# ForJadeForest/DistillCLIP

Hardware: AMD Instinct MI355X
Metric: image-text pairs/sec (distill step) (higher is better)
Workload: dtype bf16

## Files before the change

distillclip_amd/csrc/common.h:

```cpp
#pragma once
#include <hip/hip_runtime.h>
#include <stdint.h>

typedef __bf16 bf16_t;
typedef __attribute__((ext_vector_type(8))) __bf16 bf16x8;
typedef __attribute__((ext_vector_type(4))) __bf16 bf16x4;
typedef __attribute__((ext_vector_type(2))) __bf16 bf16x2;
typedef __attribute__((ext_vector_type(8))) _Float16 f16x8;
typedef __attribute__((ext_vector_type(4))) _Float16 f16x4;
typedef __attribute__((ext_vector_type(4))) short s16x4;
typedef __attribute__((ext_vector_type(4))) float f32x4;
typedef __attribute__((ext_vector_type(16))) float f32x16;
typedef __attribute__((ext_vector_type(4))) unsigned int u32x4;

#include "dclip.h"

void dclip_set_error(const char* fmt, ...);

#define DCLIP_REQUIRE(cond, ...)                 \
    do {                                          \
        if (!(cond)) {                            \
            dclip_set_error(__VA_ARGS__);         \
            return DCLIP_EINVAL;                  \
        }                                         \
// ... 20 lines not shown
    hipError_t e = hipGetLastError();
    if (e != hipSuccess) {
        dclip_explain_hip_error(what, (int)e, hipGetErrorString(e));
        return DCLIP_ELAUNCH;
    }
    return DCLIP_OK;
}

__device__ __forceinline__ float bf2f(bf16_t x) { return (float)x; }
__device__ __forceinline__ bf16_t f2bf(float x) { return (bf16_t)x; }

__device__ __forceinline__ float wave_sum(float v) {
#pragma unroll
    for (int o = 32; o > 0; o >>= 1) v += __shfl_xor(v, o);
    return v;
}
__device__ __forceinline__ float wave_max(float v) {
#pragma unroll
    for (int o = 32; o > 0; o >>= 1) v = fmaxf(v, __shfl_xor(v, o));
    return v;
}

__device__ __forceinline__ float quick_gelu_f(float x) { return x * __builtin_amdgcn_rcpf(1.f + __expf(-1.702f * x)); }
__device__ __forceinline__ float erf_tail(float ax_over_sqrt2, float phi) {
    const float t = __builtin_amdgcn_rcpf(fmaf(0.3275911f, ax_over_sqrt2, 1.f));
    float p = fmaf(1.061405429f, t, -1.453152027f);
    p = fmaf(p, t, 1.421413741f);
    p = fmaf(p, t, -0.284496736f);
    p = fmaf(p, t, 0.254829592f);
    return p * t * phi;
}
__device__ __forceinline__ float gelu_erf_f(float x) {
    const float phi = __expf(-0.5f * x * x);
    const float tail = erf_tail(fabsf(x) * 0.70710678118654752f, phi);
    const float cdf = x >= 0.f ? 1.f - 0.5f * tail : 0.5f * tail;
    return x * cdf;
}
__device__ __forceinline__ float dgelu_erf_f(float x) {
    const float phi = __expf(-0.5f * x * x);
    const float tail = erf_tail(fabsf(x) * 0.70710678118654752f, phi);
    const float cdf = x >= 0.f ? 1.f - 0.5f * tail : 0.5f * tail;
    return fmaf(x * phi, 0.3989422804014327f, cdf);
}

__device__ __forceinline__ void gelu_erf_both_f(float x, float& g, float& dg) {
    const float phi = __expf(-0.5f * x * x);
    const float tail = erf_tail(fabsf(x) * 0.70710678118654752f, phi);
    const float cdf = x >= 0.f ? 1.f - 0.5f * tail : 0.5f * tail;
    g = x * cdf;
    dg = fmaf(x * phi, 0.3989422804014327f, cdf);
}

#define DCLIP_DG_LO (-0.13f)
#define DCLIP_DG_STEP (1.26f / 255.f)
__device__ __forceinline__ unsigned dg_pack4(float a, float b, float c, float d) {
    const float inv = 255.f / 1.26f, off = 0.13f * (255.f / 1.26f);
    unsigned r = 0;
    r = __builtin_amdgcn_cvt_pk_u8_f32(__builtin_rintf(fmaf(a, inv, off)), 0, r);
    r = __builtin_amdgcn_cvt_pk_u8_f32(__builtin_rintf(fmaf(b, inv, off)), 1, r);
    r = __builtin_amdgcn_cvt_pk_u8_f32(__builtin_rintf(fmaf(c, inv, off)), 2, r);
    r = __builtin_amdgcn_cvt_pk_u8_f32(__builtin_rintf(fmaf(d, inv, off)), 3, r);
    return r;
}
__device__ __forceinline__ float dg_unpack(unsigned w, int byte) {
    return fmaf((float)((w >> (8 * byte)) & 0xffu), DCLIP_DG_STEP, DCLIP_DG_LO);
}

__device__ __forceinline__ int xcd_remap(int bid, int nwg) {
    const int q = nwg >> 3, r = nwg & 7, x = bid & 7;
// ... 3 lines not shown
```

distillclip_amd/csrc/encoder.cpp:

```cpp
#include <math.h>
#include <stdlib.h>
#include <string.h>
#include <atomic>
#include <new>
#include <vector>
#include "common.h"

namespace {

#define CK(expr)                      \
    do {                              \
        int _rc = (expr);             \
        if (_rc != DCLIP_OK) return _rc; \
    } while (0)

inline size_t up256(size_t x) { return (x + 255) & ~(size_t)255; }

struct Bump {
    char* base; size_t off;
    explicit Bump(void* b) : base((char*)b), off(0) {}
    template <class T> T* take(size_t n) {
        T* p = base ? (T*)(base + off) : nullptr;
        off += up256(n * sizeof(T));
        return p;
// ... 300 lines not shown
        dclip_set_error("dclip_encoder: clearing the backward seeds failed");
        return DCLIP_ELAUNCH;
    }
    return DCLIP_OK;
}

static int encoder_forward_impl(const dclip_encoder* e, const void* input, const bf16_t* ext_patches, int64_t B, const void* const* params,
                                const void* wcache, void* workspace, size_t ws_bytes, int training,
                                float* last_representation, float* const* rep_out, float* emb_out, int64_t tokens_eff,
                                void* st) {
    DCLIP_REQUIRE(e && (input || ext_patches) && params && wcache && workspace && last_representation, "dclip_encoder_forward: null argument");
    DCLIP_REQUIRE(B > 0, "dclip_encoder_forward: empty batch");
    const Plan& p = e->p;
    DCLIP_REQUIRE(!ext_patches || (p.image && ((uintptr_t)ext_patches % 16) == 0), "dclip_encoder_forward_patches: image towers only, 16-byte aligned rows");
    DCLIP_REQUIRE(!training || p.train, "dclip_encoder_forward: the frozen teacher tower (kind 0) is inference-only");
    DCLIP_REQUIRE(tokens_eff == 0 || (!p.train && !p.image && p.c.causal && tokens_eff > 0 && tokens_eff <= p.N && !rep_out && !emb_out),
                  "dclip_encoder_forward: tokens_eff is only valid for the causal text teacher without hidden-state export");
    Work w;
    layout(p, B, training != 0, workspace, w, tokens_eff);
    DCLIP_REQUIRE(ws_bytes >= w.bytes, "dclip_encoder_forward: workspace too small (%zu < %zu)", ws_bytes, w.bytes);
    DCLIP_REQUIRE(((uintptr_t)workspace % 256) == 0 && ((uintptr_t)wcache % 256) == 0, "dclip_encoder_forward: buffers must be 256-byte aligned");
    const bf16_t* W = (const bf16_t*)wcache;
    const int64_t N = tokens_eff ? tokens_eff : p.N, D = p.D, F = p.F, E = p.E, M = B * N, H = p.H, hd = p.hd, Np = (N + 7) & ~(int64_t)7;
    const float scale = 1.f / sqrtf((float)hd);
    const int nex = p.L * p.R;

    if (p.image) {
        const bf16_t* patches = ext_patches ? ext_patches : w.patches;
        if (!ext_patches) CK(dclip_im2row((const float*)input, w.patches, B, p.c.in_chans, p.c.resolution, p.c.patch, 1, st));
        if (p.student) {
            CK(dclip_token_table(PF(params, 3), PF(params, 2), PF(params, 1), w.tok_table, N, D, st));
            CK(gemm(patches, p.K, W + p.w_embed, p.K, w.X[0], D, M, D, p.K, nullptr, 0, nullptr, nullptr, nullptr, 0, 1, N, w.tok_table, st));
        } else {
            CK(dclip_token_table(PF(params, 2), PF(params, 1), nullptr, w.tok_table, N, D, st));
            const int sdt0 = w.h16 ? DCLIP_OUT_F16 : DCLIP_OUT_F32;
            CK(gemm(patches, p.K, W + p.w_embed, p.K, w.x0, D, M, D, p.K, nullptr, 0, nullptr, nullptr, nullptr, 0, sdt0, N, w.tok_table, st));
            CK(ln_stream(w.h16, w.x0, D, nullptr, PF(params, 3), PF(params, 4), w.X[0], D, sdt0, w.mean0, w.rstd0, M, D, st));
        }
    } else if (p.compressed) {
        CK(dclip_embed_gather((const int64_t*)input, p.N, PF(params, 0), nullptr, w.patches, 0, M, N, p.c.embed_rank, st));
        CK(dclip_token_table(PF(params, 3), nullptr, PF(params, 2), w.tok_table, N, D, st));
        CK(gemm(w.patches, p.c.embed_rank, W + p.w_embed, p.c.embed_rank, w.X[0], D, M, D, p.c.embed_rank, nullptr, 0, nullptr, nullptr, nullptr, 0, 1, N, w.tok_table, st));
    } else {
        CK(dclip_embed_gather((const int64_t*)input, p.N, PF(params, 0), PF(params, 1), w.X[0], w.h16 ? DCLIP_OUT_F16 : DCLIP_OUT_F32, M, N, D, st));
    }

// ... 9 lines not shown
            n1w = PF(params, bx.n1w); n1b = PF(params, bx.n1b); n2w = PF(params, bx.n2w); n2b = PF(params, bx.n2b);
            bq = PF(params, bx.qkvb); bp = PF(params, bx.prb); b1 = PF(params, bx.f1b); b2 = PF(params, bx.f2b);
            if (p.student && p.c.head_mix) { wl = PF(params, bx.cl); ww = PF(params, bx.cw); }
        }
        void* xin = w.X[ei];
        void* xout = w.X[ei + 1];
        const int sdt = w.h16 ? DCLIP_OUT_F16 : DCLIP_OUT_F32;
        CK(ln_stream(w.h16, xin, D, nullptr, n1w, n1b, s.h1, D, DCLIP_OUT_BF16, s.mean1, s.rstd1, M, D, st));
        CK(gemm(s.h1, D, W + bw.qkv, D, s.qkv, 3 * D, M, 3 * D, D, bq, 0, nullptr, nullptr, nullptr, 0, 0, 0, nullptr, st));
        if (!training && !wl) {
            CK(dclip_attn_fused_fwd(s.qkv, 3 * D, s.ctx, D, B, H, N, hd, scale, p.c.causal, st));
        } else {
            if (wl && mix_attn(p, N)) {
                CK(dclip_attn_mix_fwd(s.qkv, 3 * D, wl, ww, s.Rm, s.stats, B, H, N, Np, hd, scale, st));
                CK(dclip_attn_nn(s.Rm, s.qkv + 2 * D, 3 * D, s.ctx, D, B, H, N, Np, hd, 1.f, 1, st));
            } else {
                CK(dclip_attn_nt(s.qkv, 3 * D, s.qkv + D, 3 * D, s.S, 1, B, H, N, Np, hd, scale, st));
                CK(dclip_attn_softmax_fwd(s.S, wl, ww, wl ? s.P : nullptr, s.Rm, B, H, N, Np, p.c.causal, st));
                CK(dclip_attn_nn(s.Rm, s.qkv + 2 * D, 3 * D, s.ctx, D, B, H, N, Np, hd, 1.f, 0, st));
            }
        }
        CK(gemm(s.ctx, D, W + bw.proj, D, s.x_mid, D, M, D, D, bp, 0, nullptr, nullptr, xin, D, sdt, 0, nullptr, st));
        CK(ln_stream(w.h16, s.x_mid, D, nullptr, n2w, n2b, s.h2, D, DCLIP_OUT_BF16, s.mean2, s.rstd2, M, D, st));
        CK(gemm(s.h2, D, W + bw.fc1, D, s.u, F, M, F, D, b1, p.student ? (s.z ? DCLIP_ACT_GELU_SAVE : DCLIP_ACT_GELU) : (s.z ? DCLIP_ACT_QUICKGELU_SAVE : DCLIP_ACT_QUICKGELU), nullptr, s.z, nullptr, 0, 0, 0, nullptr, st));
        CK(gemm(s.u, F, W + bw.fc2, F, xout, D, M, D, F, b2, 0, nullptr, nullptr, s.x_mid, D, sdt, 0, nullptr, st));
        if (rep_out && rep_out[ei]) CK(export_stream(w.h16, xout, rep_out[ei], M * D, st));
    }

    CK(dclip_pick_index(p.image ? nullptr : (const int64_t*)input, p.N, w.pick, B, N, st));
    const int f = p.p_final;
    CK(ln_stream(w.h16, w.X[nex], D, w.pick, PF(params, f), PF(params, f + 1), w.hf, D, DCLIP_OUT_BF16, w.meanf, w.rstdf, B, D, st));
    CK(gemm(w.hf, D, W + p.w_head, D, last_representation, E, B, E, D, p.student ? PF(params, f + 3) : nullptr, 0, nullptr, nullptr, nullptr, 0, 1, 0, nullptr, st));
    if (training) {
        CK(clear_backward_seeds(p, w, M, st));
        e->seeded.store(workspace, std::memory_order_release);
    }
    return DCLIP_OK;
}

extern "C" int dclip_encoder_forward(const dclip_encoder* e, const void* input, int64_t B, const void* const* params,
                                     const void* wcache, void* workspace, size_t ws_bytes, int training,
                                     float* last_representation, float* const* rep_out, float* emb_out, int64_t tokens_eff,
                                     void* st) {
    DCLIP_REQUIRE(input, "dclip_encoder_forward: null argument");
    return encoder_forward_impl(e, input, nullptr, B, params, wcache, workspace, ws_bytes, training, last_representation, rep_out, emb_out,
                                tokens_eff, st);
}
// ... 16 lines not shown
    layout(p, B, training != 0, workspace, w);
    DCLIP_REQUIRE(ws_bytes >= w.bytes, "dclip_encoder_last_layer_output: workspace too small (%zu < %zu)", ws_bytes, w.bytes);
    const bf16_t* W = (const bf16_t*)wcache;
    const int64_t M = B * p.N, D = p.D, E = p.E;
    const int nex = p.L * p.R, f = p.p_final;
    CK(ln_stream(w.h16, w.X[nex], D, nullptr, PF(params, f), PF(params, f + 1), scratch, D, DCLIP_OUT_BF16, nullptr, nullptr, M, D, st));
    CK(gemm(scratch, D, W + p.w_head, D, out, E, M, E, D, p.student ? PF(params, f + 3) : nullptr, 0, nullptr, nullptr, nullptr, 0, 1, 0, nullptr, st));
    return DCLIP_OK;
}

static int encoder_backward_impl(const dclip_encoder* e, const void* input, const bf16_t* ext_patches, int64_t B, const void* const* params,
                                 void* const* grads, const void* wcache, void* workspace, size_t ws_bytes,
                                 const float* d_last_representation, const float* const* d_rep, const float* d_emb,
                                 dclip_bucket_cb on_bucket, void* cb_user, void* st) {
    DCLIP_REQUIRE(e && (input || ext_patches) && params && grads && wcache && workspace && d_last_representation, "dclip_encoder_backward: null argument");
    const Plan& p = e->p;
    DCLIP_REQUIRE(!ext_patches || p.image, "dclip_encoder_backward_patches: image towers only");
    DCLIP_REQUIRE(p.train, "dclip_encoder_backward: the frozen teacher tower (kind 0) has no backward");
    Work w;
    layout(p, B, true, workspace, w);
    DCLIP_REQUIRE(ws_bytes >= w.bytes, "dclip_encoder_backward: workspace too small");
    const bf16_t* W = (const bf16_t*)wcache;
    const int64_t N = p.N, D = p.D, F = p.F, E = p.E, M = B * N, H = p.H, hd = p.hd, Np = p.Np;
    const float scale = 1.f / sqrtf((float)hd);
    const int nex = p.L * p.R;
    auto GR = [&](int i) -> float* { return (float*)grads[i]; };
    hipStream_t hs = (hipStream_t)st;

    {
        void* expect = workspace;
        if (!e->seeded.compare_exchange_strong(expect, nullptr, std::memory_order_acq_rel)) CK(clear_backward_seeds(p, w, M, st));
    }
    const int f = p.p_final;
    CK(dclip_cast_bf16(d_last_representation, w.dout, B * E, st));
    if (p.student) {
        if (GR(f + 2)) CK(dclip_gemm_tn_acc(w.dout, E, w.hf, D, GR(f + 2), D, B, E, D, 1, w.tn_ws, w.tn_ws_bytes, st));
        if (GR(f + 3)) CK(dclip_colsum_acc(w.dout, E, GR(f + 3), B, E, st));
    } else if (GR(f + 2)) {
        CK(dclip_gemm_tn_acc(w.hf, D, w.dout, E, GR(f + 2), E, B, D, E, 1, w.tn_ws, w.tn_ws_bytes, st));
    }
    CK(gemm(w.dout, E, W + p.w_head_t, E, w.dh, D, B, D, E, nullptr, 0, nullptr, nullptr, nullptr, 0, 0, 0, nullptr, st));
    const int R = p.R;
    bf16_t* gb_last = w.gb_f2 + (int64_t)(R - 1) * M * D;
    CK(dclip_layernorm_bwd(w.dh, D, 0, (const float*)w.X[nex], D, w.pick, PF(params, f), w.meanf, w.rstdf, w.G, D, gb_last, D, GR(f), GR(f + 1),
                           GR(bexec(p, (nex - 1) / p.R, 0).f2b), B, D, st));
    if (on_bucket) on_bucket(cb_user, 0);

    for (int ei = nex - 1; ei >= 0; --ei) {
        const int l = ei / p.R, r = ei % p.R;
        const auto& bw = p.bw[l];
        const ExecSave& s = w.ex[ei];
        const BX bx = bexec(p, l, r);
        const float *wl = nullptr, *ww = nullptr;
        if (p.student && p.c.head_mix) { wl = PF(params, bx.cl); ww = PF(params, bx.cw); }
        bf16_t* gb_f2 = w.gb_f2 + (int64_t)r * M * D;
        bf16_t* gb_pr = w.gb_pr + (int64_t)r * M * D;
        bf16_t* dbig = w.dbig + (int64_t)r * M * F;
        bf16_t* dqkv = w.dqkv + (int64_t)r * M * 3 * D;
        const int64_t MR = (int64_t)R * M;
        const ExecSave& s0 = w.ex[ei - r];
        if (d_rep && d_rep[ei]) CK(dclip_axpy_f32(w.G, d_rep[ei], gb_f2, M * D, GR(bx.f2b), D, st));
        CK(dclip_gemm_nt(gb_f2, D, W + bw.fc2_t, D, dbig, F, M, F, D, 1.f, nullptr, DCLIP_ACT_MULAUX, s.z, nullptr, nullptr, 0, 0, 0, nullptr,
                         GR(bx.f1b), st));
        if (r == 0 && GR(bx.f2w)) CK(dclip_gemm_tn_acc(w.gb_f2, D, s0.u, F, GR(bx.f2w), F, MR, D, F, wsplits(MR, D, F), w.tn_ws, w.tn_ws_bytes, st));
        if (r == 0 && GR(bx.f1w)) CK(dclip_gemm_tn_acc(w.dbig, F, s0.h2, D, GR(bx.f1w), D, MR, F, D, wsplits(MR, F, D), w.tn_ws, w.tn_ws_bytes, st));
        CK(gemm(dbig, F, W + bw.fc1_t, F, w.dh, D, M, D, F, nullptr, 0, nullptr, nullptr, nullptr, 0, 0, 0, nullptr, st));
        CK(dclip_layernorm_bwd(w.dh, D, 0, (const float*)s.x_mid, D, nullptr, PF(params, bx.n2w), s.mean2, s.rstd2, w.G, D, gb_pr, D, GR(bx.n2w), GR(bx.n2b),
                               GR(bx.prb), M, D, st));
        if (r == 0 && GR(bx.prw)) CK(dclip_gemm_tn_acc(w.gb_pr, D, s0.ctx, D, GR(bx.prw), D, MR, D, D, wsplits(MR, D, D), w.tn_ws, w.tn_ws_bytes, st));
        bf16_t* dctx = w.dh;
        CK(gemm(gb_pr, D, W + bw.proj_t, D, dctx, D, M, D, D, nullptr, 0, nullptr, nullptr, nullptr, 0, 0, 0, nullptr, st));
        const int blk = (wl && mix_attn(p, N)) ? 1 : 0;
        CK(dclip_attn_tn(s.Rm, dctx, D, dqkv + 2 * D, 3 * D, B, H, N, Np, hd, 1.f, blk, st));
        if (wl && mix_attn(p, N)) {
            float* gl = GR(bx.cl) ? GR(bx.cl) : w.wg_dummy;
            float* gw = GR(bx.cw) ? GR(bx.cw) : w.wg_dummy + H * H;
            CK(dclip_attn_mix_bwd(s.qkv, 3 * D, dctx, D, wl, ww, s.stats, w.dS, gl, gw, w.mix_ws, w.mix_ws_bytes, B, H, N, Np, hd, scale, st));
        } else {
            CK(dclip_attn_nt(dctx, D, s.qkv + 2 * D, 3 * D, w.dR, 0, B, H, N, Np, hd, 1.f, st));
            CK(dclip_attn_softmax_bwd(w.dR, s.P, s.S, 0, wl, ww, w.dS, wl ? GR(bx.cl) : nullptr,
                                      wl ? GR(bx.cw) : nullptr, B, H, N, Np, st));
        }
        CK(dclip_attn_nn(w.dS, s.qkv + D, 3 * D, dqkv, 3 * D, B, H, N, Np, hd, scale, blk, st));
        CK(dclip_attn_tn(w.dS, s.qkv, 3 * D, dqkv + D, 3 * D, B, H, N, Np, hd, scale, blk, st));
        if (r == 0 && GR(bx.qkvw)) CK(dclip_gemm_tn_acc(w.dqkv, 3 * D, s0.h1, D, GR(bx.qkvw), D, MR, 3 * D, D, wsplits(MR, 3 * D, D), w.tn_ws, w.tn_ws_bytes, st));
// ... 78 lines not shown
```

distillclip_amd/csrc/gemm.hip:

```cpp

#include "gemm_common.h"
#include <atomic>

using namespace dgemm;

namespace {

constexpr int TILE_BYTES = (BM / 16) * (BK / 32) * SUB;
constexpr int CLD = BN + 4;
constexpr int NT_LDS = (4 * TILE_BYTES > BM * CLD * 4) ? 4 * TILE_BYTES : BM * CLD * 4;


__device__ __forceinline__ void stage_operand(const bf16_t* __restrict__ G, int64_t ld, int row0, int rows_max,
                                              int k0, char* lds_tile, int wave, int lane) {
    const int L = lane * 16;
    const int X = swz(L);
    const int r = X >> 6, c = (X >> 4) & 3;
#pragma unroll
    for (int s = 0; s < 4; ++s) {
        const int sub = wave * 4 + s;
        const int rb = sub >> 1, kb = sub & 1;
        int row = row0 + rb * 16 + r;
        row = row < rows_max ? row : rows_max - 1;
        const bf16_t* src = G + (int64_t)row * ld + (k0 + kb * 32 + c * 8);
// ... 77 lines not shown
    float csum[8];
#pragma unroll
    for (int e = 0; e < 8; ++e) csum[e] = 0.f;
#pragma unroll
    for (int it = 0; it < 8; ++it) {
        const int rl = (tid >> 4) + it * 16;
        const int row = m0 + rl;
        if (row >= p.M || !col_ok) break;
        float v[8];
        {
            const float4 c0 = *(const float4*)(cs + rl * CLD + cc), c1 = *(const float4*)(cs + rl * CLD + cc + 4);
            v[0] = c0.x; v[1] = c0.y; v[2] = c0.z; v[3] = c0.w; v[4] = c1.x; v[5] = c1.y; v[6] = c1.z; v[7] = c1.w;
        }
#pragma unroll
        for (int e = 0; e < 8; ++e) v[e] = v[e] * p.alpha + bias[e];
        if (p.row_group > 0) {
            const float* ra = p.rowadd + (int64_t)(row % p.row_group) * p.N + col;
            const float4 a0 = *(const float4*)ra, a1 = *(const float4*)(ra + 4);
            v[0] += a0.x; v[1] += a0.y; v[2] += a0.z; v[3] += a0.w; v[4] += a1.x; v[5] += a1.y; v[6] += a1.z; v[7] += a1.w;
        }
        const int64_t o = (int64_t)row * p.ldc + col;
        {
            EpiSide sd;
            epilogue_load_side<ACT, OUT>(p, o, (int64_t)row * p.ldr + col, sd);
            float zero[8] = {0.f, 0.f, 0.f, 0.f, 0.f, 0.f, 0.f, 0.f}, unused[8];
            GemmNT q = p;
            q.alpha = 1.f; q.row_group = 0; q.colsum = nullptr;
            epilogue_vec8<ACT, OUT, 0>(q, v, row, col, o, (int64_t)row * p.ldr + col, zero, unused, sd);
        }
#pragma unroll
        for (int e = 0; e < 8; ++e) csum[e] += v[e];
    }
    if (p.colsum) {
        __syncthreads();
#pragma unroll
        for (int e = 0; e < 8; ++e) cs[(tid >> 4) * CLD + cc + e] = csum[e];
        __syncthreads();
        if (tid < BN && n0 + tid < p.N) {
            float x = 0.f;
#pragma unroll
            for (int r = 0; r < 16; ++r) x += cs[r * CLD + tid];
            unsafeAtomicAdd(p.colsum + n0 + tid, x);
        }
    }
}

constexpr int HT = 16384;
// ... 173 lines not shown
                    acc[RH + i][2 + j] = __builtin_amdgcn_mfma_f32_16x16x32_bf16(b1[j][kb], af[i][kb], acc[RH + i][2 + j], 0, 0, 0);
            }
        __builtin_amdgcn_s_setprio(0);
        __builtin_amdgcn_s_barrier();
    }
    if (wr == 0) __builtin_amdgcn_s_barrier();
    stamp(2);
    const int m0c = m0, n0c = n0;
    const int g = ln >> 4, rl = ln & 15;

    const int colb = n0c + wc * 64 + g * 8;
    float bias[2][8], csum[2][8];
#pragma unroll
    for (int jp = 0; jp < 2; ++jp) {
#pragma unroll
        for (int e = 0; e < 8; ++e) { bias[jp][e] = 0.f; csum[jp][e] = 0.f; }
        const int col = colb + jp * 32;
        if (p.bias && col < p.N) {
            const float4 q0 = *(const float4*)(p.bias + col), q1 = *(const float4*)(p.bias + col + 4);
            bias[jp][0] = q0.x; bias[jp][1] = q0.y; bias[jp][2] = q0.z; bias[jp][3] = q0.w;
            bias[jp][4] = q1.x; bias[jp][5] = q1.y; bias[jp][6] = q1.z; bias[jp][7] = q1.w;
        }
    }
    constexpr bool OUT_F32 = OUT == 1;
    constexpr bool SIDE = OUT != 0 || ACT == 3 || ACT == 4;
    constexpr int NU = 2 * MI;
    constexpr int BU = !SIDE ? NU : (OUT_F32 ? ((ACT == 3 || ACT == 4) ? 4 : (MI == 8 ? 8 : (MI == 6 ? 6 : 5))) : (MI == 10 ? 10 : NU));
    static_assert(NU % BU == 0, "batch size must divide the unit count");
    EpiSide side[SIDE ? BU : 1];
    const int row0 = m0c + wr * AROWS + rl;
    const int64_t o0 = (int64_t)row0 * p.ldc + colb, r0off = (int64_t)row0 * p.ldr + colb;
    const int64_t ostep = 16 * p.ldc, rstep = 16 * p.ldr;
    const bool full = m0c + BMT <= p.M && n0c + 256 <= p.N;
    auto run_units = [&](auto mode_tag) {
        constexpr int MODE = decltype(mode_tag)::value;
#pragma unroll
        for (int ub = 0; ub < NU; ub += BU) {
            if (SIDE) {
#pragma unroll
                for (int u = ub; u < ub + BU; ++u) {
                    const int i = u >> 1, jp = u & 1;
                    if (full || (row0 + i * 16 < p.M && colb + jp * 32 < p.N))
                        epilogue_load_side<ACT, OUT>(p, o0 + i * ostep + jp * 32, r0off + i * rstep + jp * 32, side[u - ub]);
                }
            }
#pragma unroll
            for (int u = ub; u < ub + BU; ++u) {
                const int i = u >> 1, jp = u & 1;
                const int row = row0 + i * 16, col = colb + jp * 32;
                if (full || (row < p.M && col < p.N)) {
                    float v[8];
#pragma unroll
                    for (int r = 0; r < 4; ++r) { v[r] = acc[i][2 * jp][r]; v[4 + r] = acc[i][2 * jp + 1][r]; }
                    epilogue_vec8<ACT, OUT, MODE>(p, v, row, col, o0 + i * ostep + jp * 32, r0off + i * rstep + jp * 32, bias[jp], csum[jp],
                                                      side[SIDE ? u - ub : 0]);
                }
            }
        }
    };
    const bool lean = p.row_group == 0 && ((ACT == 5 || ACT == 6) ? p.aux_out != nullptr : p.aux_out == nullptr) && (OUT != 0 ? p.residual != nullptr : p.residual == nullptr);
    if constexpr (OUT != 0) {
        if (lean) run_units(std::integral_constant<int, 3>{});
        else run_units(std::integral_constant<int, 0>{});
    } else if constexpr (ACT == 3 || ACT == 4) {
        if (lean && p.colsum) run_units(std::integral_constant<int, 2>{});
        else run_units(std::integral_constant<int, 0>{});
    } else {
        if (lean && !p.colsum) run_units(std::integral_constant<int, 1>{});
        else if (lean) run_units(std::integral_constant<int, 2>{});
        else run_units(std::integral_constant<int, 0>{});
    }
    if (OUT == 0 && p.colsum) {
        float* cs = (float*)smem;
#pragma unroll
        for (int jp = 0; jp < 2; ++jp)
#pragma unroll
            for (int e = 0; e < 8; ++e) {
                const float x = row16_sum(csum[jp][e]);
                if (rl == 0) cs[wr * 256 + wc * 64 + jp * 32 + g * 8 + e] = x;
            }
        WAIT_LGKM0();
        __builtin_amdgcn_s_barrier();
        const int tc = wave * 64 + ln;
        if (tc < 256 && n0c + tc < p.N) unsafeAtomicAdd(p.colsum + n0c + tc, cs[tc] + cs[256 + tc]);
    }
    stamp(3);
    if (p.clk && blockIdx.x == 0 && tid == 0) { p.clk[2] = __builtin_amdgcn_s_memtime(); p.clk[3] = __builtin_amdgcn_s_memrealtime(); }
}

constexpr int TP = 128, TQ = 128, TC = 64;
constexpr int TROW = 288;
constexpr int TTILE = TC * TROW;

// ... 568 lines not shown
    else hipLaunchKernelGGL((gemm_nt_kernel<ACT, 0>), dim3(grid), dim3(256), lds, st, p);
    return dclip_check_launch("dclip_gemm_nt");
}

unsigned long long* g_gemm_stamps = nullptr;
std::atomic<long long> g_tn_atomic_fallbacks{0};

}

extern "C" int dclip_trace_gemm_stamps(void* buf) { g_gemm_stamps = (unsigned long long*)buf; return 0; }
extern "C" int64_t dclip_trace_gemm_clock(void* buf, int64_t cap) {
    const long long n = g_clock_count.exchange(0, std::memory_order_relaxed);
    g_clock_cap.store(buf ? (long long)cap : 0, std::memory_order_relaxed);
    g_clock_buf.store((unsigned long long*)buf, std::memory_order_release);
    return (int64_t)n;
}
extern "C" int64_t dclip_gemm_tn_atomic_fallbacks(void) { return (int64_t)g_tn_atomic_fallbacks.load(std::memory_order_relaxed); }

extern "C" int dclip_gemm_nt(const void* A, int64_t lda, const void* B, int64_t ldb, void* C, int64_t ldc,
                             int64_t M, int64_t N, int64_t K, float alpha, const float* bias, int act,
                             const void* aux_in, void* aux_out, const void* residual, int64_t ldr, int out_dtype,
                             int64_t row_group, const float* rowadd, float* colsum_acc, void* stream) {
    DCLIP_REQUIRE(A && B && C, "dclip_gemm_nt: null operand");
    DCLIP_REQUIRE(M > 0 && N > 0 && K > 0, "dclip_gemm_nt: empty problem M=%ld N=%ld K=%ld", (long)M, (long)N, (long)K);
    DCLIP_REQUIRE(K % BK == 0, "dclip_gemm_nt: K=%ld must be a multiple of %d", (long)K, BK);
    DCLIP_REQUIRE(lda % 8 == 0 && ldb % 8 == 0 && ((uintptr_t)A % 16) == 0 && ((uintptr_t)B % 16) == 0,
                  "dclip_gemm_nt: operand rows must be 16-byte aligned (lda=%ld ldb=%ld)", (long)lda, (long)ldb);
    DCLIP_REQUIRE(N % 8 == 0 && ldc % 8 == 0 && ((uintptr_t)C % 16) == 0, "dclip_gemm_nt: N and ldc must be multiples of 8 and C 16-byte aligned (N=%ld ldc=%ld)", (long)N, (long)ldc);
    DCLIP_REQUIRE(out_dtype >= 0 && out_dtype <= 2, "dclip_gemm_nt: bad output dtype %d (0 bf16, 1 f32, 2 f16)", out_dtype);
    DCLIP_REQUIRE(!residual || (ldr % (out_dtype == 2 ? 8 : 4) == 0 && ((uintptr_t)residual % 16) == 0), "dclip_gemm_nt: residual rows must be 16-byte aligned");
    DCLIP_REQUIRE(act >= 0 && act <= 6, "dclip_gemm_nt: bad activation code %d", act);
    DCLIP_REQUIRE(out_dtype != 2 || act == 0, "dclip_gemm_nt: f16 output needs act = DCLIP_ACT_NONE");
    DCLIP_REQUIRE((act != DCLIP_ACT_DGELU && act != DCLIP_ACT_MULAUX) || aux_in, "dclip_gemm_nt: DGELU / MULAUX need aux_in");
    DCLIP_REQUIRE(!aux_in || ((uintptr_t)aux_in % 16) == 0, "dclip_gemm_nt: aux_in must be 16-byte aligned");
    DCLIP_REQUIRE(!aux_out || ((uintptr_t)aux_out % 16) == 0, "dclip_gemm_nt: aux_out must be 16-byte aligned");
    DCLIP_REQUIRE(row_group == 0 || rowadd, "dclip_gemm_nt: row_group needs rowadd");
    DCLIP_REQUIRE(M < (1LL << 31) && N < (1LL << 31), "dclip_gemm_nt: dimension overflow");
    GemmNT p;
    p.A = (const bf16_t*)A; p.lda = lda; p.B = (const bf16_t*)B; p.ldb = ldb; p.C = C; p.ldc = ldc;
    p.M = (int)M; p.N = (int)N; p.K = (int)K; p.alpha = alpha; p.bias = bias;
    p.aux_in = aux_in; p.aux_out = aux_out; p.residual = residual; p.ldr = ldr;
    p.row_group = (int)row_group; p.rowadd = rowadd; p.colsum = colsum_acc;
    p.tiles_m = (int)((M + BM - 1) / BM); p.tiles_n = (int)((N + BN - 1) / BN);
    p.stamps = g_gemm_stamps;
    p.group_n = 1 << 30;
    p.clk = nullptr;
    hipStream_t st = (hipStream_t)stream;
    const int out_f32 = out_dtype == 1;
    const double aux_b = (act == DCLIP_ACT_MULAUX || act == DCLIP_ACT_GELU_SAVE || act == DCLIP_ACT_QUICKGELU_SAVE) ? 1.0 : 2.0;
    TraceScope tr(DCLIP_TRACE_GEMM_NT, 2.0 * (double)M * (double)N * (double)K,
                  2.0 * ((double)M * K + (double)N * K) + ((out_f32 ? 4.0 : 2.0) + (residual ? (out_dtype == 2 ? 2.0 : 4.0) : 0.0) + (aux_in ? aux_b : 0.0) + (aux_out ? aux_b : 0.0)) * (double)M * N,
                  stream, (int)M, (int)N, (int)K,
                  act + 8 * (out_f32 != 0) + 16 * (residual != nullptr) + 32 * (colsum_acc != nullptr) + 64 * (out_dtype == 2));
    switch (act) {
        case 0: return launch_nt<0>(p, out_dtype, st);
        case 1: return launch_nt<1>(p, out_dtype, st);
        case 2: return launch_nt<2>(p, out_dtype, st);
        case 3: return launch_nt<3>(p, out_dtype, st);
        case 4: return launch_nt<4>(p, out_dtype, st);
        case 5: return launch_nt<5>(p, out_dtype, st);
        default: return launch_nt<6>(p, out_dtype, st);
    }
}

extern "C" size_t dclip_gemm_tn_workspace_bytes(void) { return (size_t)384 * 65536 * sizeof(float); }

extern "C" int dclip_gemm_tn_acc(const void* A, int64_t lda, const void* B, int64_t ldb, float* dW, int64_t ldo,
                                 int64_t M, int64_t P, int64_t Q, int splits, void* workspace, size_t ws_bytes, void* stream) {
// ... 59 lines not shown
```

distillclip_amd/csrc/gemm_common.h:

```cpp
#pragma once
#include <math.h>
#include <stdlib.h>
#include "common.h"
#include <type_traits>

namespace dgemm {

constexpr int BM = 128, BN = 128, BK = 64;
constexpr int SUB = 1024;

struct GemmNT {
    const bf16_t* A; int64_t lda;
    const bf16_t* B; int64_t ldb;
    void* C; int64_t ldc;
    int M, N, K;
    float alpha;
    const float* bias;
    const void* aux_in;
    void* aux_out;
    const void* residual; int64_t ldr;
    int row_group; const float* rowadd;
    float* colsum;
    int tiles_m, tiles_n;
    unsigned long long* stamps;
    int group_n;
    unsigned long long* clk;
};

__device__ __forceinline__ int swz(int x) { return x ^ (((x >> 9) & 1) << 5); }

typedef __attribute__((address_space(3))) void lds_void;
typedef __attribute__((address_space(1))) const void gbl_void;

struct EpiSide {
    float4 r0, r1;
    f16x8 rh;
    bf16x8 z;
    uint2 zq;
};

template <int ACT, int OUT>
__device__ __forceinline__ void epilogue_load_side(const GemmNT& p, int64_t o, int64_t orr, EpiSide& sd) {
    if (OUT == 1 && p.residual) {
        const float* rp = (const float*)p.residual + orr;
        sd.r0 = *(const float4*)rp; sd.r1 = *(const float4*)(rp + 4);
    }
    if (OUT == 2 && p.residual) sd.rh = *(const f16x8*)((const _Float16*)p.residual + orr);
    if (ACT == 3) sd.z = *(const bf16x8*)((const bf16_t*)p.aux_in + o);
    if (ACT == 4) sd.zq = *(const uint2*)((const uint8_t*)p.aux_in + o);
}

template <int ACT, int OUT, int MODE = 0>
__device__ __forceinline__ void epilogue_vec8(const GemmNT& p, float (&v)[8], int row, int col, int64_t o, int64_t orr,
                                              const float (&bias)[8], float (&csum)[8], const EpiSide& sd) {
    constexpr bool LEAN = MODE != 0;
#pragma unroll
    for (int e = 0; e < 8; ++e) v[e] = v[e] * p.alpha + bias[e];
    if (!LEAN && p.row_group > 0) {
        const float* ra = p.rowadd + (int64_t)(row % p.row_group) * p.N + col;
        const float4 a0 = *(const float4*)ra, a1 = *(const float4*)(ra + 4);
        v[0] += a0.x; v[1] += a0.y; v[2] += a0.z; v[3] += a0.w; v[4] += a1.x; v[5] += a1.y; v[6] += a1.z; v[7] += a1.w;
    }
    if (!LEAN && ACT != 5 && ACT != 6 && p.aux_out) {
        bf16x8 z;
#pragma unroll
        for (int e = 0; e < 8; ++e) z[e] = f2bf(v[e]);
        *(bf16x8*)((bf16_t*)p.aux_out + o) = z;
    }
    if (ACT == 1) {
#pragma unroll
        for (int e = 0; e < 8; ++e) v[e] = quick_gelu_f(v[e]);
    }
    if (ACT == 2) {
#pragma unroll
        for (int e = 0; e < 8; ++e) v[e] = gelu_erf_f(v[e]);
    }
    if (ACT == 3) {
        const bf16x8 z = sd.z;
#pragma unroll
        for (int e = 0; e < 8; ++e) v[e] *= dgelu_erf_f(bf2f(z[e]));
    }
    if (ACT == 4) {
        const uint2 q = sd.zq;
        v[0] *= dg_unpack(q.x, 0); v[1] *= dg_unpack(q.x, 1); v[2] *= dg_unpack(q.x, 2); v[3] *= dg_unpack(q.x, 3);
        v[4] *= dg_unpack(q.y, 0); v[5] *= dg_unpack(q.y, 1); v[6] *= dg_unpack(q.y, 2); v[7] *= dg_unpack(q.y, 3);
    }
    if (ACT == 5) {
        float dg[8];
#pragma unroll
        for (int e = 0; e < 8; ++e) {
            float g;
            gelu_erf_both_f(v[e], g, dg[e]);
            v[e] = g;
        }
        if (LEAN || p.aux_out) *(uint2*)((uint8_t*)p.aux_out + o) = uint2{dg_pack4(dg[0], dg[1], dg[2], dg[3]), dg_pack4(dg[4], dg[5], dg[6], dg[7])};
    }
    if (ACT == 6) {
        float dg[8];
#pragma unroll
        for (int e = 0; e < 8; ++e) {
            const float sg = __builtin_amdgcn_rcpf(1.f + __expf(-1.702f * v[e]));
            dg[e] = fmaf(1.702f * v[e] * sg, 1.f - sg, sg);
            v[e] *= sg;
        }
        if (LEAN || p.aux_out) *(uint2*)((uint8_t*)p.aux_out + o) = uint2{dg_pack4(dg[0], dg[1], dg[2], dg[3]), dg_pack4(dg[4], dg[5], dg[6], dg[7])};
    }
    if (MODE == 3 || (!LEAN && p.residual)) {
        if (OUT == 2) {
            const f16x8 r = sd.rh;
#pragma unroll
            for (int e = 0; e < 8; ++e) v[e] += (float)r[e];
        } else {
            float4 r0, r1;
            if (OUT == 1) { r0 = sd.r0; r1 = sd.r1; }
            else {
                const float* rp = (const float*)p.residual + orr;
                r0 = *(const float4*)rp; r1 = *(const float4*)(rp + 4);
            }
            v[0] += r0.x; v[1] += r0.y; v[2] += r0.z; v[3] += r0.w; v[4] += r1.x; v[5] += r1.y; v[6] += r1.z; v[7] += r1.w;
        }
    }
    if (OUT == 1) {
        float* cp = (float*)p.C + o;
        *(float4*)cp = float4{v[0], v[1], v[2], v[3]};
        *(float4*)(cp + 4) = float4{v[4], v[5], v[6], v[7]};
    } else if (OUT == 2) {
        f16x8 ov;
#pragma unroll
// ... 19 lines not shown
```

distillclip_amd/ops.py:

```python
import torch

from ._lib import lib

ACT = {'none': 0, None: 0, 'quickgelu': 1, 'gelu': 2, 'dgelu': 3, 'mulaux': 4, 'gelu_save': 5, 'quickgelu_save': 6}
OUT_DTYPE = {torch.bfloat16: 0, torch.float32: 1, torch.float16: 2}
DG_LO, DG_STEP = -0.13, 1.26 / 255.0


def _p(t):
    return 0 if t is None else t.data_ptr()


def _stream():
    return torch.cuda.current_stream().cuda_stream


def _chk(*ts):
    for t in ts:
        if t is not None and not t.is_cuda:
            raise RuntimeError('distillclip_amd ops need CUDA(HIP) tensors; there is no CPU fallback')


def gemm_nt(a, b, *, bias=None, act=None, aux_in=None, aux_out=None, residual=None, out=None, out_dtype=torch.bfloat16,
            alpha=1.0, row_group=0, rowadd=None, out_rows=None, colsum=None):
    _chk(a, b, bias, aux_in, aux_out, residual, out, rowadd)
    assert a.dtype == torch.bfloat16 and b.dtype == torch.bfloat16 and a.dim() == 2 and b.dim() == 2
    assert a.stride(1) == 1 and b.stride(1) == 1
    M, K = a.shape
    N = b.shape[0]
    if out is None:
        rows = out_rows if out_rows is not None else M
        out = torch.empty((rows, N), dtype=out_dtype, device=a.device)
    assert out.stride(1) == 1
    ldr = residual.stride(0) if residual is not None else 0
    if act in ('gelu_save', 'quickgelu_save') and aux_out is not None:
        assert aux_out.dtype == torch.uint8 and aux_out.stride(0) == out.stride(0)
    if act == 'mulaux':
        assert aux_in.dtype == torch.uint8 and aux_in.stride(0) == out.stride(0)
    if residual is not None:
        assert residual.dtype == (torch.float16 if out.dtype == torch.float16 else torch.float32)
    lib().dclip_gemm_nt(_p(a), a.stride(0), _p(b), b.stride(0), _p(out), out.stride(0), M, N, K, float(alpha),
                        _p(bias), ACT[act], _p(aux_in), _p(aux_out), _p(residual), ldr,
                        OUT_DTYPE[out.dtype], row_group, _p(rowadd), _p(colsum), _stream())
    return out


_TN_WS = {}


def _tn_workspace(device):
    key = (device, _stream())
    ws = _TN_WS.get(key)
    if ws is None:
        ws = _TN_WS[key] = torch.empty(lib().dclip_gemm_tn_workspace_bytes(), dtype=torch.uint8, device=device)
    return ws


def gemm_tn_acc(a, b, dw, splits=4, workspace=True):
    _chk(a, b, dw)
    assert a.dtype == torch.bfloat16 and b.dtype == torch.bfloat16 and dw.dtype == torch.float32
    M, P = a.shape
    Q = b.shape[1]
    assert b.shape[0] == M and tuple(dw.shape) == (P, Q) and dw.stride(1) == 1
    ws = _tn_workspace(a.device) if workspace else None
    lib().dclip_gemm_tn_acc(_p(a), a.stride(0), _p(b), b.stride(0), _p(dw), dw.stride(0), M, P, Q, splits, _p(ws),
# ... 173 lines not shown
```

include/dclip.h:

```cpp
#ifndef DCLIP_H
#define DCLIP_H
#include <stddef.h>
#include <stdint.h>
#ifdef __cplusplus
extern "C" {
#endif

#define DCLIP_OK 0
#define DCLIP_EINVAL (-1)
#define DCLIP_ELAUNCH (-2)

int dclip_version(void);
int dclip_runtime_check(void);
const char* dclip_arch(void);
const char* dclip_last_error_string(void);

#define DCLIP_ACT_NONE 0
#define DCLIP_ACT_QUICKGELU 1
#define DCLIP_ACT_GELU 2
#define DCLIP_ACT_DGELU 3
#define DCLIP_ACT_MULAUX 4
#define DCLIP_ACT_GELU_SAVE 5
#define DCLIP_ACT_QUICKGELU_SAVE 6
#define DCLIP_OUT_BF16 0
#define DCLIP_OUT_F32 1
#define DCLIP_OUT_F16 2

int dclip_gemm_nt(const void* A, int64_t lda, const void* B, int64_t ldb, void* C, int64_t ldc,
                  int64_t M, int64_t N, int64_t K, float alpha, const float* bias, int act,
                  const void* aux_in, void* aux_out, const void* residual, int64_t ldr, int out_dtype,
                  int64_t row_group, const float* rowadd, float* colsum_acc, void* stream);

size_t dclip_gemm_tn_workspace_bytes(void);
int64_t dclip_gemm_tn_atomic_fallbacks(void);
int dclip_gemm_tn_acc(const void* A, int64_t lda, const void* B, int64_t ldb, float* dW, int64_t ldo,
                      int64_t M, int64_t P, int64_t Q, int splits, void* workspace, size_t ws_bytes, void* stream);

int dclip_colsum_acc(const void* X, int64_t ld, float* db, int64_t M, int64_t N, void* stream);

int dclip_layernorm_fwd(const float* x, int64_t ldx, const int32_t* row_index, const float* gamma, const float* beta,
                        void* y, int64_t ldy, int out_f32, float* mean, float* rstd, int64_t M, int64_t D, float eps,
                        void* stream);
int dclip_layernorm_fwd_f16(const void* x, int64_t ldx, const int32_t* row_index, const float* gamma, const float* beta,
                            void* y, int64_t ldy, int out_dtype, float* mean, float* rstd, int64_t M, int64_t D, float eps,
                            void* stream);
int dclip_layernorm_bwd(const void* dy, int64_t lddy, int dy_f32, const float* x, int64_t ldx, const int32_t* row_index,
// ... 135 lines not shown
```

Before: 16850.

## Tile the saved GELU-derivative aux buffer so epilogues use 16-byte accesses

```diff
diff --git a/distillclip_amd/csrc/common.h b/distillclip_amd/csrc/common.h
--- a/distillclip_amd/csrc/common.h
+++ b/distillclip_amd/csrc/common.h
@@ -66,6 +66,7 @@
 }
 
 __device__ __forceinline__ float quick_gelu_f(float x) { return x * __builtin_amdgcn_rcpf(1.f + __expf(-1.702f * x)); }
+__device__ __forceinline__ float gauss_f(float x) { return __builtin_amdgcn_exp2f(x * x * (-0.5f * 1.44269504088896341f)); }
 __device__ __forceinline__ float erf_tail(float ax_over_sqrt2, float phi) {
     const float t = __builtin_amdgcn_rcpf(fmaf(0.3275911f, ax_over_sqrt2, 1.f));
     float p = fmaf(1.061405429f, t, -1.453152027f);
@@ -75,20 +76,20 @@
     return p * t * phi;
 }
 __device__ __forceinline__ float gelu_erf_f(float x) {
-    const float phi = __expf(-0.5f * x * x);
+    const float phi = gauss_f(x);
     const float tail = erf_tail(fabsf(x) * 0.70710678118654752f, phi);
     const float cdf = x >= 0.f ? 1.f - 0.5f * tail : 0.5f * tail;
     return x * cdf;
 }
 __device__ __forceinline__ float dgelu_erf_f(float x) {
-    const float phi = __expf(-0.5f * x * x);
+    const float phi = gauss_f(x);
     const float tail = erf_tail(fabsf(x) * 0.70710678118654752f, phi);
     const float cdf = x >= 0.f ? 1.f - 0.5f * tail : 0.5f * tail;
     return fmaf(x * phi, 0.3989422804014327f, cdf);
 }
 
 __device__ __forceinline__ void gelu_erf_both_f(float x, float& g, float& dg) {
-    const float phi = __expf(-0.5f * x * x);
+    const float phi = gauss_f(x);
     const float tail = erf_tail(fabsf(x) * 0.70710678118654752f, phi);
     const float cdf = x >= 0.f ? 1.f - 0.5f * tail : 0.5f * tail;
     g = x * cdf;
diff --git a/distillclip_amd/csrc/encoder.cpp b/distillclip_amd/csrc/encoder.cpp
--- a/distillclip_amd/csrc/encoder.cpp
+++ b/distillclip_amd/csrc/encoder.cpp
@@ -346,6 +346,7 @@
     DCLIP_REQUIRE(((uintptr_t)workspace % 256) == 0 && ((uintptr_t)wcache % 256) == 0, "dclip_encoder_forward: buffers must be 256-byte aligned");
     const bf16_t* W = (const bf16_t*)wcache;
     const int64_t N = tokens_eff ? tokens_eff : p.N, D = p.D, F = p.F, E = p.E, M = B * N, H = p.H, hd = p.hd, Np = (N + 7) & ~(int64_t)7;
+    const int zt = F % 16 == 0 ? DCLIP_AUX_TILED : 0;
     const float scale = 1.f / sqrtf((float)hd);
     const int nex = p.L * p.R;
 
@@ -401,7 +402,7 @@
         }
         CK(gemm(s.ctx, D, W + bw.proj, D, s.x_mid, D, M, D, D, bp, 0, nullptr, nullptr, xin, D, sdt, 0, nullptr, st));
         CK(ln_stream(w.h16, s.x_mid, D, nullptr, n2w, n2b, s.h2, D, DCLIP_OUT_BF16, s.mean2, s.rstd2, M, D, st));
-        CK(gemm(s.h2, D, W + bw.fc1, D, s.u, F, M, F, D, b1, p.student ? (s.z ? DCLIP_ACT_GELU_SAVE : DCLIP_ACT_GELU) : (s.z ? DCLIP_ACT_QUICKGELU_SAVE : DCLIP_ACT_QUICKGELU), nullptr, s.z, nullptr, 0, 0, 0, nullptr, st));
+        CK(gemm(s.h2, D, W + bw.fc1, D, s.u, F, M, F, D, b1, p.student ? (s.z ? DCLIP_ACT_GELU_SAVE | zt : DCLIP_ACT_GELU) : (s.z ? DCLIP_ACT_QUICKGELU_SAVE | zt : DCLIP_ACT_QUICKGELU), nullptr, s.z, nullptr, 0, 0, 0, nullptr, st));
         CK(gemm(s.u, F, W + bw.fc2, F, xout, D, M, D, F, b2, 0, nullptr, nullptr, s.x_mid, D, sdt, 0, nullptr, st));
         if (rep_out && rep_out[ei]) CK(export_stream(w.h16, xout, rep_out[ei], M * D, st));
     }
@@ -464,6 +465,7 @@
     DCLIP_REQUIRE(ws_bytes >= w.bytes, "dclip_encoder_backward: workspace too small");
     const bf16_t* W = (const bf16_t*)wcache;
     const int64_t N = p.N, D = p.D, F = p.F, E = p.E, M = B * N, H = p.H, hd = p.hd, Np = p.Np;
+    const int zt = F % 16 == 0 ? DCLIP_AUX_TILED : 0;
     const float scale = 1.f / sqrtf((float)hd);
     const int nex = p.L * p.R;
     auto GR = [&](int i) -> float* { return (float*)grads[i]; };
@@ -502,7 +504,7 @@
         const int64_t MR = (int64_t)R * M;
         const ExecSave& s0 = w.ex[ei - r];
         if (d_rep && d_rep[ei]) CK(dclip_axpy_f32(w.G, d_rep[ei], gb_f2, M * D, GR(bx.f2b), D, st));
-        CK(dclip_gemm_nt(gb_f2, D, W + bw.fc2_t, D, dbig, F, M, F, D, 1.f, nullptr, DCLIP_ACT_MULAUX, s.z, nullptr, nullptr, 0, 0, 0, nullptr,
+        CK(dclip_gemm_nt(gb_f2, D, W + bw.fc2_t, D, dbig, F, M, F, D, 1.f, nullptr, DCLIP_ACT_MULAUX | zt, s.z, nullptr, nullptr, 0, 0, 0, nullptr,
                          GR(bx.f1b), st));
         if (r == 0 && GR(bx.f2w)) CK(dclip_gemm_tn_acc(w.gb_f2, D, s0.u, F, GR(bx.f2w), F, MR, D, F, wsplits(MR, D, F), w.tn_ws, w.tn_ws_bytes, st));
         if (r == 0 && GR(bx.f1w)) CK(dclip_gemm_tn_acc(w.dbig, F, s0.h2, D, GR(bx.f1w), D, MR, F, D, wsplits(MR, F, D), w.tn_ws, w.tn_ws_bytes, st));
diff --git a/distillclip_amd/csrc/gemm.hip b/distillclip_amd/csrc/gemm.hip
--- a/distillclip_amd/csrc/gemm.hip
+++ b/distillclip_amd/csrc/gemm.hip
@@ -123,7 +123,7 @@
         const int64_t o = (int64_t)row * p.ldc + col;
         {
             EpiSide sd;
-            epilogue_load_side<ACT, OUT>(p, o, (int64_t)row * p.ldr + col, sd);
+            epilogue_load_side<ACT, OUT>(p, o, (int64_t)row * p.ldr + col, p.aux_tiled ? aux_tiled_off(o, col, p.N) : o, sd);
             float zero[8] = {0.f, 0.f, 0.f, 0.f, 0.f, 0.f, 0.f, 0.f}, unused[8];
             GemmNT q = p;
             q.alpha = 1.f; q.row_group = 0; q.colsum = nullptr;
@@ -343,30 +343,54 @@
             bias[jp][4] = q1.x; bias[jp][5] = q1.y; bias[jp][6] = q1.z; bias[jp][7] = q1.w;
         }
     }
+#pragma unroll
+    for (int jp = 0; jp < 2; ++jp)
+#pragma unroll
+        for (int e = 0; e < 8; ++e) asm volatile("" : "+v"(bias[jp][e]));
     constexpr bool OUT_F32 = OUT == 1;
     constexpr bool SIDE = OUT != 0 || ACT == 3 || ACT == 4;
     constexpr int NU = 2 * MI;
     constexpr int BU = !SIDE ? NU : (OUT_F32 ? ((ACT == 3 || ACT == 4) ? 4 : (MI == 8 ? 8 : (MI == 6 ? 6 : 5))) : (MI == 10 ? 10 : NU));
     static_assert(NU % BU == 0, "batch size must divide the unit count");
-    EpiSide side[SIDE ? BU : 1];
+    EpiSide side[SIDE ? (ACT == 4 ? NU : BU) : 1];
     const int row0 = m0c + wr * AROWS + rl;
     const int64_t o0 = (int64_t)row0 * p.ldc + colb, r0off = (int64_t)row0 * p.ldr + colb;
     const int64_t ostep = 16 * p.ldc, rstep = 16 * p.ldr;
     const bool full = m0c + BMT <= p.M && n0c + 256 <= p.N;
-    auto run_units = [&](auto mode_tag) {
+    const bool wide_aux = (ACT == 4 || ACT == 5 || ACT == 6) && p.aux_tiled && n0c + wc * 64 + 64 <= p.N;
+    constexpr bool SAVE = ACT == 5 || ACT == 6;
+    auto aux_unit_off = [&](int mode, int64_t o, int col) { return mode == 0 && p.aux_tiled ? aux_tiled_off(o, col, p.N) : o; };
+    auto run_units = [&](auto mode_tag, auto wide_tag) {
         constexpr int MODE = decltype(mode_tag)::value;
-#pragma unroll
-        for (int ub = 0; ub < NU; ub += BU) {
+        constexpr bool wide = decltype(wide_tag)::value;
+        constexpr int BW = ACT == 4 && wide ? NU : BU;
+#pragma unroll
+        for (int ub = 0; ub < NU; ub += BW) {
             if (SIDE) {
 #pragma unroll
-                for (int u = ub; u < ub + BU; ++u) {
+                for (int u = ub; u < ub + BW; ++u) {
                     const int i = u >> 1, jp = u & 1;
-                    if (full || (row0 + i * 16 < p.M && colb + jp * 32 < p.N))
-                        epilogue_load_side<ACT, OUT>(p, o0 + i * ostep + jp * 32, r0off + i * rstep + jp * 32, side[u - ub]);
+                    if constexpr (ACT == 4 && wide) {
+#if DCLIP_DIAG_EPI == 1
+                        if (jp == 0) { side[u - ub].zq = uint2{(unsigned)u * 0x01010101u, 0u}; side[u + 1 - ub].zq = uint2{0u, (unsigned)i}; }
+#else
+                        if (jp == 0) {
+                            const bool ok = full || row0 + i * 16 < p.M;
+                            const uint4 q = *(const uint4*)((const uint8_t*)p.aux_in + (ok ? o0 + i * ostep + g * 8 : 0));
+                            side[u - ub].zq = uint2{q.x, q.y};
+                            side[u + 1 - ub].zq = uint2{q.z, q.w};
+                        }
+#endif
+                    } else {
+                        const bool ok = full || (row0 + i * 16 < p.M && colb + jp * 32 < p.N);
+                        const int64_t o = ok ? o0 + i * ostep + jp * 32 : 0;
+                        epilogue_load_side<ACT, OUT>(p, o, ok ? r0off + i * rstep + jp * 32 : 0, aux_unit_off(MODE, o, ok ? colb + jp * 32 : 0), side[u - ub]);
+                    }
                 }
             }
-#pragma unroll
-            for (int u = ub; u < ub + BU; ++u) {
+            uint2 dq[2];
+#pragma unroll
+            for (int u = ub; u < ub + BW; ++u) {
                 const int i = u >> 1, jp = u & 1;
                 const int row = row0 + i * 16, col = colb + jp * 32;
                 if (full || (row < p.M && col < p.N)) {
@@ -374,22 +398,35 @@
 #pragma unroll
                     for (int r = 0; r < 4; ++r) { v[r] = acc[i][2 * jp][r]; v[4 + r] = acc[i][2 * jp + 1][r]; }
                     epilogue_vec8<ACT, OUT, MODE>(p, v, row, col, o0 + i * ostep + jp * 32, r0off + i * rstep + jp * 32, bias[jp], csum[jp],
-                                                      side[SIDE ? u - ub : 0]);
+                                                      side[SIDE ? u - ub : 0], SAVE ? &dq[jp] : nullptr);
                 }
-            }
-        }
+#if DCLIP_DIAG_EPI != 1
+                if (SAVE && (MODE != 0 || p.aux_out) && (full || (row < p.M && col < p.N))) {
+                    uint8_t* z = (uint8_t*)p.aux_out;
+                    if constexpr (wide) { if (jp == 1) *(uint4*)(z + o0 + i * ostep + g * 8) = uint4{dq[0].x, dq[0].y, dq[1].x, dq[1].y}; }
+                    else *(uint2*)(z + aux_unit_off(MODE, o0 + i * ostep + jp * 32, col)) = dq[jp];
+                }
+#endif
+            }
+        }
+    };
+    auto run = [&](auto mode_tag) {
+        if constexpr ((ACT == 4 || ACT == 5 || ACT == 6) && decltype(mode_tag)::value != 0) {
+            if (wide_aux) { run_units(mode_tag, std::true_type{}); return; }
+        }
+        run_units(mode_tag, std::false_type{});
     };
     const bool lean = p.row_group == 0 && ((ACT == 5 || ACT == 6) ? p.aux_out != nullptr : p.aux_out == nullptr) && (OUT != 0 ? p.residual != nullptr : p.residual == nullptr);
     if constexpr (OUT != 0) {
-        if (lean) run_units(std::integral_constant<int, 3>{});
-        else run_units(std::integral_constant<int, 0>{});
+        if (lean) run(std::integral_constant<int, 3>{});
+        else run(std::integral_constant<int, 0>{});
     } else if constexpr (ACT == 3 || ACT == 4) {
-        if (lean && p.colsum) run_units(std::integral_constant<int, 2>{});
-        else run_units(std::integral_constant<int, 0>{});
+        if (lean && p.colsum) run(std::integral_constant<int, 2>{});
+        else run(std::integral_constant<int, 0>{});
     } else {
-        if (lean && !p.colsum) run_units(std::integral_constant<int, 1>{});
-        else if (lean) run_units(std::integral_constant<int, 2>{});
-        else run_units(std::integral_constant<int, 0>{});
+        if (lean && !p.colsum) run(std::integral_constant<int, 1>{});
+        else if (lean) run(std::integral_constant<int, 2>{});
+        else run(std::integral_constant<int, 0>{});
     }
     if (OUT == 0 && p.colsum) {
         float* cs = (float*)smem;
@@ -1004,6 +1041,11 @@
                              const void* aux_in, void* aux_out, const void* residual, int64_t ldr, int out_dtype,
                              int64_t row_group, const float* rowadd, float* colsum_acc, void* stream) {
     DCLIP_REQUIRE(A && B && C, "dclip_gemm_nt: null operand");
+    const int aux_tiled = (act & DCLIP_AUX_TILED) != 0;
+    act &= ~DCLIP_AUX_TILED;
+    DCLIP_REQUIRE(!aux_tiled || act == DCLIP_ACT_MULAUX || act == DCLIP_ACT_GELU_SAVE || act == DCLIP_ACT_QUICKGELU_SAVE,
+                  "dclip_gemm_nt: DCLIP_AUX_TILED needs act = DCLIP_ACT_MULAUX, DCLIP_ACT_GELU_SAVE or DCLIP_ACT_QUICKGELU_SAVE (act %d)", act);
+    DCLIP_REQUIRE(!aux_tiled || ldc % 16 == 0, "dclip_gemm_nt: DCLIP_AUX_TILED needs ldc %% 16 == 0 (ldc=%ld)", (long)ldc);
     DCLIP_REQUIRE(M > 0 && N > 0 && K > 0, "dclip_gemm_nt: empty problem M=%ld N=%ld K=%ld", (long)M, (long)N, (long)K);
     DCLIP_REQUIRE(K % BK == 0, "dclip_gemm_nt: K=%ld must be a multiple of %d", (long)K, BK);
     DCLIP_REQUIRE(lda % 8 == 0 && ldb % 8 == 0 && ((uintptr_t)A % 16) == 0 && ((uintptr_t)B % 16) == 0,
@@ -1026,6 +1068,7 @@
     p.tiles_m = (int)((M + BM - 1) / BM); p.tiles_n = (int)((N + BN - 1) / BN);
     p.stamps = g_gemm_stamps;
     p.group_n = 1 << 30;
+    p.aux_tiled = aux_tiled;
     p.clk = nullptr;
     hipStream_t st = (hipStream_t)stream;
     const int out_f32 = out_dtype == 1;
diff --git a/distillclip_amd/csrc/gemm_common.h b/distillclip_amd/csrc/gemm_common.h
--- a/distillclip_amd/csrc/gemm_common.h
+++ b/distillclip_amd/csrc/gemm_common.h
@@ -25,7 +25,14 @@
     unsigned long long* stamps;
     int group_n;
     unsigned long long* clk;
+    int aux_tiled;
 };
+
+__device__ __forceinline__ int64_t aux_tiled_off(int64_t o, int col, int N) {
+    const int c = col & 63, q = c >> 3;
+    if (col - c + 64 > N) return o;
+    return o - c + (((q & 3) << 1) | (q >> 2)) * 8;
+}
 
 __device__ __forceinline__ int swz(int x) { return x ^ (((x >> 9) & 1) << 5); }
 
@@ -39,20 +46,37 @@
     uint2 zq;
 };
 
+#ifndef DCLIP_DIAG_EPI
+#define DCLIP_DIAG_EPI 0
+#endif
+#if DCLIP_DIAG_EPI == 1
+#define DIAG_AUX_STORE(...) do { const uint2 q_ = __VA_ARGS__; asm volatile("" :: "v"(q_.x), "v"(q_.y)); } while (0)
+#else
+#define DIAG_AUX_STORE(...) do {                                                                                      \
+        const uint2 q_ = __VA_ARGS__;                                                                                  \
+        if (dq_out) *dq_out = q_;                                                                                      \
+        else if (LEAN || p.aux_out) *(uint2*)((uint8_t*)p.aux_out + (p.aux_tiled ? aux_tiled_off(o, col, p.N) : o)) = q_; \
+    } while (0)
+#endif
+
 template <int ACT, int OUT>
-__device__ __forceinline__ void epilogue_load_side(const GemmNT& p, int64_t o, int64_t orr, EpiSide& sd) {
+__device__ __forceinline__ void epilogue_load_side(const GemmNT& p, int64_t o, int64_t orr, int64_t oaux, EpiSide& sd) {
     if (OUT == 1 && p.residual) {
         const float* rp = (const float*)p.residual + orr;
         sd.r0 = *(const float4*)rp; sd.r1 = *(const float4*)(rp + 4);
     }
     if (OUT == 2 && p.residual) sd.rh = *(const f16x8*)((const _Float16*)p.residual + orr);
     if (ACT == 3) sd.z = *(const bf16x8*)((const bf16_t*)p.aux_in + o);
-    if (ACT == 4) sd.zq = *(const uint2*)((const uint8_t*)p.aux_in + o);
+#if DCLIP_DIAG_EPI == 1
+    if (ACT == 4) sd.zq = uint2{(unsigned)o * 0x01010101u, (unsigned)orr * 0x01010101u};
+#else
+    if (ACT == 4) sd.zq = *(const uint2*)((const uint8_t*)p.aux_in + oaux);
+#endif
 }
 
 template <int ACT, int OUT, int MODE = 0>
 __device__ __forceinline__ void epilogue_vec8(const GemmNT& p, float (&v)[8], int row, int col, int64_t o, int64_t orr,
-                                              const float (&bias)[8], float (&csum)[8], const EpiSide& sd) {
+                                              const float (&bias)[8], float (&csum)[8], const EpiSide& sd, uint2* dq_out = nullptr) {
     constexpr bool LEAN = MODE != 0;
 #pragma unroll
     for (int e = 0; e < 8; ++e) v[e] = v[e] * p.alpha + bias[e];
@@ -90,10 +114,14 @@
 #pragma unroll
         for (int e = 0; e < 8; ++e) {
             float g;
+#if DCLIP_DIAG_EPI == 2
+            g = quick_gelu_f(v[e]); dg[e] = g;
+#else
             gelu_erf_both_f(v[e], g, dg[e]);
+#endif
             v[e] = g;
         }
-        if (LEAN || p.aux_out) *(uint2*)((uint8_t*)p.aux_out + o) = uint2{dg_pack4(dg[0], dg[1], dg[2], dg[3]), dg_pack4(dg[4], dg[5], dg[6], dg[7])};
+        DIAG_AUX_STORE(uint2{dg_pack4(dg[0], dg[1], dg[2], dg[3]), dg_pack4(dg[4], dg[5], dg[6], dg[7])});
     }
     if (ACT == 6) {
         float dg[8];
@@ -103,7 +131,7 @@
             dg[e] = fmaf(1.702f * v[e] * sg, 1.f - sg, sg);
             v[e] *= sg;
         }
-        if (LEAN || p.aux_out) *(uint2*)((uint8_t*)p.aux_out + o) = uint2{dg_pack4(dg[0], dg[1], dg[2], dg[3]), dg_pack4(dg[4], dg[5], dg[6], dg[7])};
+        DIAG_AUX_STORE(uint2{dg_pack4(dg[0], dg[1], dg[2], dg[3]), dg_pack4(dg[4], dg[5], dg[6], dg[7])});
     }
     if (MODE == 3 || (!LEAN && p.residual)) {
         if (OUT == 2) {
diff --git a/distillclip_amd/ops.py b/distillclip_amd/ops.py
--- a/distillclip_amd/ops.py
+++ b/distillclip_amd/ops.py
@@ -22,7 +22,7 @@
 
 
 def gemm_nt(a, b, *, bias=None, act=None, aux_in=None, aux_out=None, residual=None, out=None, out_dtype=torch.bfloat16,
-            alpha=1.0, row_group=0, rowadd=None, out_rows=None, colsum=None):
+            alpha=1.0, row_group=0, rowadd=None, out_rows=None, colsum=None, aux_tiled=False):
     _chk(a, b, bias, aux_in, aux_out, residual, out, rowadd)
     assert a.dtype == torch.bfloat16 and b.dtype == torch.bfloat16 and a.dim() == 2 and b.dim() == 2
     assert a.stride(1) == 1 and b.stride(1) == 1
@@ -40,7 +40,7 @@
     if residual is not None:
         assert residual.dtype == (torch.float16 if out.dtype == torch.float16 else torch.float32)
     lib().dclip_gemm_nt(_p(a), a.stride(0), _p(b), b.stride(0), _p(out), out.stride(0), M, N, K, float(alpha),
-                        _p(bias), ACT[act], _p(aux_in), _p(aux_out), _p(residual), ldr,
+                        _p(bias), ACT[act] | (256 if aux_tiled else 0), _p(aux_in), _p(aux_out), _p(residual), ldr,
                         OUT_DTYPE[out.dtype], row_group, _p(rowadd), _p(colsum), _stream())
     return out
 
diff --git a/include/dclip.h b/include/dclip.h
--- a/include/dclip.h
+++ b/include/dclip.h
@@ -22,6 +22,7 @@
 #define DCLIP_ACT_MULAUX 4
 #define DCLIP_ACT_GELU_SAVE 5
 #define DCLIP_ACT_QUICKGELU_SAVE 6
+#define DCLIP_AUX_TILED 256
 #define DCLIP_OUT_BF16 0
 #define DCLIP_OUT_F32 1
 #define DCLIP_OUT_F16 2
```

Result: no change. 16900, median of 6 (+0.3%).
